# mpkuse/solve_keyframe_pose_graph

Measured on AMD Instinct MI355X. Metric: LM iters/sec + final chi2 vs Ceres, 100k-pose/300k-edge SE(3) graph, higher is better.
Workload: dtype f64

## Files before the change

solve_keyframe_pose_graph_amd/csrc/pgo_internal.hpp:

```cpp
#pragma once
#include <hip/hip_runtime.h>
#include <stdint.h>

#include "pgo_device_math.hpp"

#define PGO_HIPCHK(err, expr)                                                                      \
    do {                                                                                           \
        hipError_t e__ = (expr);                                                                   \
        if (e__ != hipSuccess) {                                                                   \
            (err) = std::string(#expr) + ": " + hipGetErrorString(e__);                            \
            return e__ == hipErrorOutOfMemory ? PGO_ERR_OUT_OF_MEMORY : PGO_ERR_HIP;               \
        }                                                                                          \
    } while (0)

namespace pgo {

constexpr int TILE = 64;
constexpr int REL_DOUBLES = 78;
constexpr int SW_DOUBLES = 86;
constexpr int K1_WAVES = 4;
constexpr int WIN_MAX = 72;
constexpr int WIN_STRIDE = 80;
constexpr int MAX_PARTIALS = 1024;
constexpr int CG_MAX_GRID = 1024;
// ... 70 lines not shown
    double* cen;
    double* d;
    double* Ac;
    double* rc;
    double* yc;
    const int64_t* blk_ptr;
    const int32_t* blk_ab;
    const int64_t* contrib;
    const int32_t* agg_free;
    float* Acf;
};

constexpr int MG_MAX_LEVELS = 12;
constexpr int MG_TILE_ROWS = 32;
struct MgLevelDev {
    int32_t n, n_next, tiles, n_ps;
    int64_t nnzb;
    const int64_t* rowptr; const int32_t* col; double* val;
    const int64_t* g_ptr; const int64_t* g_ent;
    double* Dinv;
    double* pos; double* d;
    const int32_t* parent; const int32_t* agg_ptr; const int4* tile_info; const int2* tile_rows;
    double* r; double* x; double* xt; double* xf;
    float* valf;
    int32_t smoothed, n_w;
    int32_t seg_shift, pad3_;
    const int32_t* ps_rowptr; const int32_t* ps_col; const int32_t* w_rowptr; const int32_t* w_col; const int64_t* psT_ptr; const int64_t* psT_ent;
    double* ps_val; double* w_val;
    double* t; double* u; double* y; const double* zero;
    double* dlump;
    const int32_t* row_of; const int32_t* tr_of;
    const int32_t* ps_row; const int32_t* w_row;
    float* rt_valf; float* r_valf;
    const int2* rt_rows; const int2* rT_rows; const int32_t* rT_col; const int32_t* rT_of_w; const int32_t* ps_of_w;
    int32_t rT_tiles, rT_seg_shift;
    int32_t tile0, tiles_own, rT_row0, rT_row1;
    int32_t su_row0, su_row1, su_ps0, su_ps1, su_w0, su_w1, n_su_prod, pad4_;
    int64_t su_blk0, su_blk1;
    const int32_t* su_prod;
};
struct MgDev {
    int32_t n_levels;
    int32_t n1;
    const int32_t* agg0;
    const int32_t* mem0_ptr; const int32_t* mem0;
    double* d0;
    const int4* blk_tab;
    const double* inv_cnt;
    int32_t a0, a1;
    const int32_t* g0_slots; int32_t n_g0, pad_;
};
constexpr int MG_BLOCK0 = 64;

struct CgDev {
    double* val; float* Lf; double* Dtot; double* b;
    double* x; double* r; double* r2; double* z; double* p; double* p2; double* q;
    double* part_pq;
    double* part_rz;
    int32_t extra_rz;
    int32_t pad_;
    double* scal;
    int32_t* flags;
};

void launch_k1(const GraphDev& G, const double* pose8, const double* sw, bool want_jacobian, double* partials , int* n_partials, hipStream_t st);
void launch_prior(const GraphDev& G, const double* pose8, bool want_jacobian, double* partial_cost , hipStream_t st);
void launch_k2(const GraphDev& G, const LinDev& L, bool want_offdiag, hipStream_t st, const MfDev* F = nullptr );
void launch_scale_init(const GraphDev& G, const LinDev& L, const ScaleDev& Sc, int jacobi_scaling, hipStream_t st);
// ... 93 lines not shown
```

solve_keyframe_pose_graph_amd/csrc/pgo_mg_host.hpp:

```cpp
#pragma once
#include <algorithm>
#include <cmath>
#include <cstdint>
#include <numeric>
#include <utility>
#include <cstdlib>
#include <cstring>
#include <thread>
#include <atomic>
#include <new>
#include <vector>
#include <chrono>
#include <cstdio>
#define PGO_MG_T0() auto t_mg_ = std::chrono::steady_clock::now()
#define PGO_MG_T(what) do { if (pgo_mg::timing()) { auto n_ = std::chrono::steady_clock::now(); std::fprintf(stderr, "[pgo] hierarchy (host): %-28s %7.2f ms\n", what, std::chrono::duration<double, std::milli>(n_ - t_mg_).count()); t_mg_ = n_; } } while (0)

namespace pgo_mg { inline bool& timing() { static thread_local bool on = false; return on; } }

namespace pgo_mg {

struct HostLevel {
    int32_t n = 0;
    std::vector<int64_t> rowptr;
    std::vector<int32_t> col;
    std::vector<int64_t> g_ptr;
    std::vector<int64_t> g_ent;
    std::vector<int32_t> parent;
    std::vector<int32_t> agg_ptr;
    std::vector<int32_t> tile_agg0;
    int seg = 1;
    bool smoothed = false;
    std::vector<int32_t> ps_rowptr, ps_col;
    std::vector<int32_t> w_rowptr, w_col;
    std::vector<int64_t> psT_ptr, psT_ent;
    std::vector<int32_t> ps_of_w;
    std::vector<int32_t> rT_rowptr, rT_col;
    std::vector<int32_t> rT_of_w;
    int rT_seg = 1;
    std::vector<int32_t> own_ptr;
    std::vector<int32_t> tile_ptr;
    bool distributed = false;
};

struct Hierarchy {
    std::vector<HostLevel> L;
    bool fine_smoothed = false;
    HostLevel F;
    std::vector<int32_t> agg0;
    std::vector<int32_t> mem0_ptr, mem0;
    int world = 1;
};

struct Owners {
    const std::vector<uint64_t>* touch_mask = nullptr;
    const std::vector<int32_t>* owner = nullptr;
    int world = 1;
    int32_t dist_min_rows = 8192;
};

struct WEdge { int32_t u, v; double w; };

template <class Fn>
inline void parallel_ranges(int32_t n, int parts, Fn fn) {
    if (parts < 1) parts = 1;
    if (parts == 1 || n < 2048) { fn(0, 0, n); return; }
    std::atomic<bool> helper_failed{false};
    struct Joiner { std::vector<std::thread> th; ~Joiner() { for (std::thread& t : th) if (t.joinable()) t.join(); } } j;
    const int32_t step = (n + parts - 1) / parts;
    for (int k = 0; k + 1 < parts; ++k) {
        const int32_t lo = std::min<int64_t>((int64_t)k * step, n), hi = std::min<int64_t>((int64_t)(k + 1) * step, n);
        bool started = false;
// ... 121 lines not shown
    const std::vector<int32_t>* sc1; const std::vector<int32_t>* sc2;
};

struct BuildCache {
    bool valid = false;
    std::vector<int32_t> agg0_prov; int32_t n1 = 0;
    HostLevel L1prov;
    std::vector<WEdge> rel1;
    std::vector<int32_t> sw_u, sw_v;
    std::vector<int64_t> sw_ptr; std::vector<int32_t> sw_edge;
    std::vector<int32_t> own1_prov;
};

inline void permute_level1(const HostLevel& P, int32_t n, const std::vector<int32_t>& newid, HostLevel& out) {
    std::vector<int32_t> old_of((size_t)n);
    for (int32_t i = 0; i < n; ++i) old_of[newid[i]] = i;
    out.rowptr.assign((size_t)n + 1, 0); out.col.resize(P.col.size()); out.g_ptr.assign(P.col.size() + 1, 0); out.g_ent.resize(P.g_ent.size());
    int64_t kb = 0, ge = 0;
    std::vector<std::pair<int32_t, int64_t>> row;
    for (int32_t r = 0; r < n; ++r) {
        const int32_t o = old_of[r];
        row.clear();
        for (int64_t k = P.rowptr[o]; k < P.rowptr[(size_t)o + 1]; ++k) { const int32_t c = newid[P.col[k]]; row.push_back({c == r ? -1 : c, k}); }
        std::sort(row.begin(), row.end());
        for (const auto& ck : row) {
            out.col[(size_t)kb] = ck.first < 0 ? r : ck.first;
            out.g_ptr[(size_t)kb] = ge;
            for (int64_t g = P.g_ptr[ck.second]; g < P.g_ptr[(size_t)ck.second + 1]; ++g) out.g_ent[(size_t)ge++] = P.g_ent[g];
            ++kb;
        }
        out.rowptr[(size_t)r + 1] = kb;
    }
    out.g_ptr[(size_t)kb] = ge;
}

inline void smoothed_structure(HostLevel& A, HostLevel& B, const std::vector<uint8_t>* ps_keep = nullptr) {
    A.smoothed = true;
    const int32_t n = A.n, nb = B.n;
    const int nth = host_threads();
    auto rows_in_parallel = [&](int32_t rows, std::vector<int32_t>& rowptr_out, std::vector<int32_t>& col_out, auto row_fn ) {
        std::vector<std::vector<int32_t>> part_cols((size_t)nth), part_len((size_t)nth);
        parallel_ranges(rows, nth, [&](int part, int32_t lo, int32_t hi) {
            std::vector<int32_t> tmp, stamp((size_t)nb, -1);
            std::vector<int32_t>& pc = part_cols[(size_t)part]; std::vector<int32_t>& pl = part_len[(size_t)part];
            pl.reserve((size_t)(hi - lo));
            for (int32_t i = lo; i < hi; ++i) { tmp.clear(); row_fn(i, tmp, stamp); pc.insert(pc.end(), tmp.begin(), tmp.end()); pl.push_back((int32_t)tmp.size()); }
        });
        rowptr_out.assign((size_t)rows + 1, 0); col_out.clear();
        int32_t r = 0;
        for (int k = 0; k < nth; ++k) {
            for (int32_t len : part_len[(size_t)k]) { rowptr_out[(size_t)r + 1] = rowptr_out[r] + len; ++r; }
            col_out.insert(col_out.end(), part_cols[(size_t)k].begin(), part_cols[(size_t)k].end());
        }
    };
    rows_in_parallel(n, A.ps_rowptr, A.ps_col, [&](int32_t i, std::vector<int32_t>& tmp, std::vector<int32_t>&) {
        if (A.parent[i] < 0) return;
        for (int64_t k = A.rowptr[i]; k < A.rowptr[(size_t)i + 1]; ++k) { if (ps_keep && !(*ps_keep)[(size_t)k]) continue; const int32_t a = A.parent[A.col[k]]; if (a >= 0) tmp.push_back(a); }
        std::sort(tmp.begin(), tmp.end()); tmp.erase(std::unique(tmp.begin(), tmp.end()), tmp.end());
    });
    rows_in_parallel(n, A.w_rowptr, A.w_col, [&](int32_t i, std::vector<int32_t>& tmp, std::vector<int32_t>& stamp) {
        if (A.parent[i] < 0) return;
        for (int64_t k = A.rowptr[i]; k < A.rowptr[(size_t)i + 1]; ++k) {
            const int32_t j = A.col[k];
            for (int32_t sl = A.ps_rowptr[j]; sl < A.ps_rowptr[(size_t)j + 1]; ++sl) { const int32_t c = A.ps_col[sl]; if (stamp[c] != i) { stamp[c] = i; tmp.push_back(c); } }
        }
        std::sort(tmp.begin(), tmp.end());
// ... 1 lines not shown
    A.psT_ptr.assign((size_t)nb + 1, 0);
    for (int32_t c : A.ps_col) A.psT_ptr[(size_t)c + 1]++;
    for (int32_t a = 0; a < nb; ++a) A.psT_ptr[(size_t)a + 1] += A.psT_ptr[a];
    A.psT_ent.resize(A.ps_col.size());
    { std::vector<int64_t> fill(A.psT_ptr.begin(), A.psT_ptr.end() - 1);
      for (int32_t i = 0; i < n; ++i) for (int32_t sl = A.ps_rowptr[i]; sl < A.ps_rowptr[(size_t)i + 1]; ++sl) A.psT_ent[(size_t)fill[A.ps_col[sl]]++] = ((int64_t)i << 32) | (int64_t)sl; }
    {
        std::vector<int32_t> brow, bcol;
        rows_in_parallel(nb, brow, bcol, [&](int32_t a, std::vector<int32_t>& tmp, std::vector<int32_t>& stamp) {
            std::vector<int32_t> un;
            for (int64_t e = A.psT_ptr[a]; e < A.psT_ptr[(size_t)a + 1]; ++e) {
                const int32_t i = (int32_t)(A.psT_ent[e] >> 32);
                for (int32_t sl = A.w_rowptr[i]; sl < A.w_rowptr[(size_t)i + 1]; ++sl) { const int32_t c = A.w_col[sl]; if (stamp[c] != a) { stamp[c] = a; un.push_back(c); } }
            }
            std::sort(un.begin(), un.end());
            tmp.push_back(a);
            for (int32_t c : un) if (c != a) tmp.push_back(c);
        });
        B.rowptr.assign(brow.begin(), brow.end()); B.col.swap(bcol);
    }
    B.g_ptr.assign(B.col.size() + 1, 0); B.g_ent.clear();
    A.ps_of_w.assign(A.w_col.size(), -1);
    for (int32_t i = 0; i < n; ++i) {
        int32_t ps = A.ps_rowptr[i]; const int32_t pe = A.ps_rowptr[(size_t)i + 1];
        for (int32_t k = A.w_rowptr[i]; k < A.w_rowptr[(size_t)i + 1] && ps < pe; ++k) if (A.w_col[k] == A.ps_col[ps]) A.ps_of_w[(size_t)k] = ps++;
    }
    A.rT_rowptr.assign((size_t)nb + 1, 0);
    for (int32_t c : A.w_col) A.rT_rowptr[(size_t)c + 1]++;
    for (int32_t a = 0; a < nb; ++a) A.rT_rowptr[(size_t)a + 1] += A.rT_rowptr[a];
    A.rT_col.resize(A.w_col.size()); A.rT_of_w.resize(A.w_col.size());
    { std::vector<int32_t> fill(A.rT_rowptr.begin(), A.rT_rowptr.end() - 1);
      for (int32_t i = 0; i < n; ++i) for (int32_t k = A.w_rowptr[i]; k < A.w_rowptr[(size_t)i + 1]; ++k) { const int32_t sl = fill[A.w_col[k]]++; A.rT_col[(size_t)sl] = i; A.rT_of_w[(size_t)k] = sl; } }
    {
        const double mean_row = (double)A.w_col.size() / (double)std::max(1, nb);
        static const double rt_blocks_per_group = []() {
            const char* m = std::getenv("PGO_ENABLE_DEBUG_HOOKS"); const char* e = std::getenv("PGO_DEBUG_RT_SEG_BLOCKS");
            const double v = (m && m[0] == '1' && m[1] == 0 && e) ? std::atof(e) : 0.0; return v >= 1.0 && v <= 64.0 ? v : 5.0; }();
        A.rT_seg = 1;
        while (A.rT_seg < 8 && mean_row > rt_blocks_per_group * A.rT_seg) A.rT_seg *= 2;
    }
}

inline bool build_hierarchy(int64_t N, const std::vector<uint8_t>& node_free, const std::vector<int32_t>& rc1, const std::vector<int32_t>& rc2, const double* rel_w, int rel_w_stride,
                            const std::vector<int32_t>& sc1, const std::vector<int32_t>& sc2, const double* sw_weight ,
                            int passes0, int passes, int dense_max, int tile_rows, int max_levels, Hierarchy& H, bool level0_follows_switchable = true, int level0_block = 0,
                            const LocalContrib* local = nullptr, int smoothed_levels = 0 ,
                            double loop_discount = 0.0 ,
                            BuildCache* cache = nullptr ,
                            const std::vector<int64_t>* fine_rowptr = nullptr, const std::vector<int32_t>* fine_col = nullptr ,
                            const Owners* owners = nullptr ,
                            const std::vector<uint8_t>* fine_keep = nullptr ) {
    H = Hierarchy{};
    const bool owned = owners && owners->touch_mask && owners->owner && owners->world > 1;
    const int world = owned ? owners->world : 1;
    H.world = world;
    auto kf_owner = [&](int64_t g) { return (*owners->owner)[(size_t)g]; };
    PGO_MG_T0();
    const int64_t Er = (int64_t)rc1.size(), Es = (int64_t)sc1.size();
    BuildCache own_cache;
    BuildCache& Cc = (cache && !level0_follows_switchable) ? *cache : own_cache;
    auto collapse = [](const std::vector<WEdge>& in, const std::vector<int32_t>& par) {
        std::vector<WEdge> out;
        out.reserve(in.size());
        for (const WEdge& e : in) { const int32_t u = par[e.u], v = par[e.v]; if (u >= 0 && v >= 0 && u != v) out.push_back({u, v, e.w}); }
        return out;
    };
    if (!Cc.valid) {
        std::vector<WEdge> rel_edges;
        rel_edges.reserve((size_t)Er);
        for (int64_t e = 0; e < Er; ++e) if (node_free[rc1[e]] && node_free[rc2[e]]) {
            const double w = rel_w[(size_t)rel_w_stride * e];
            if (owned && kf_owner(rc1[e]) != kf_owner(rc2[e])) continue;
            if (w * w > 1e-8) rel_edges.push_back({rc1[e], rc2[e], w * w});
// ... 204 lines not shown
    H.mem0.resize((size_t)H.mem0_ptr[n1]);
    { std::vector<int32_t> fill(H.mem0_ptr.begin(), H.mem0_ptr.end() - 1);
      for (int64_t i = 0; i < N; ++i) if (H.agg0[i] >= 0) H.mem0[(size_t)fill[H.agg0[i]]++] = (int32_t)i; }
    PGO_MG_T("numbering + member lists");
    permute_level1(Cc.L1prov, n1, newid_above, H.L[0]);
    PGO_MG_T("permute level 1");
    if (fine_rowptr && fine_col && !local) {
        H.fine_smoothed = true;
        H.F = HostLevel{};
        H.F.n = (int32_t)N; H.F.rowptr = *fine_rowptr; H.F.col = *fine_col; H.F.parent = H.agg0;
        HostLevel B1; B1.n = n1;
        smoothed_structure(H.F, B1, fine_keep);
        H.L[0].rowptr.swap(B1.rowptr); H.L[0].col.swap(B1.col); H.L[0].g_ptr.swap(B1.g_ptr); H.L[0].g_ent.clear();
        PGO_MG_T("fine-level smoothed structure");
    }
    for (size_t l = 0; l + 1 < H.L.size(); ++l) {
        HostLevel& A = H.L[l];
        HostLevel& B = H.L[l + 1];
        if ((int)l < smoothed_levels) { smoothed_structure(A, B); continue; }
        std::vector<std::pair<int64_t, int64_t>> trip;
        trip.reserve(A.col.size());
        for (int32_t r = 0; r < A.n; ++r)
            for (int64_t k = A.rowptr[r]; k < A.rowptr[(size_t)r + 1]; ++k)
                trip.push_back({(int64_t)A.parent[r] * B.n + A.parent[A.col[k]], ((int64_t)r << 32) | k});
        build_blocks(B.n, trip, B);
    }
    PGO_MG_T("upper-level structures");
    for (size_t l = 0; l + 1 < H.L.size(); ++l) {
        HostLevel& Lv = H.L[l];
        const double mean_row = (double)Lv.col.size() / (double)std::max(1, Lv.n);
        int max_agg = 1;
        const int32_t n_next = H.L[l + 1].n;
        for (int32_t a = 0; a < n_next; ++a) max_agg = std::max(max_agg, Lv.agg_ptr[(size_t)a + 1] - Lv.agg_ptr[a]);
        Lv.seg = 1;
        static const double blocks_per_group = []() {
            const char* m = std::getenv("PGO_ENABLE_DEBUG_HOOKS"); const char* e = std::getenv("PGO_DEBUG_SEG_BLOCKS");
            const double v = (m && m[0] == '1' && m[1] == 0 && e) ? std::atof(e) : 0.0; return v >= 1.0 && v <= 64.0 ? v : 5.0; }();
        while (Lv.seg < 8 && mean_row > blocks_per_group * Lv.seg) Lv.seg *= 2;
        while (Lv.seg > 1 && tile_rows / Lv.seg < max_agg) Lv.seg /= 2;
        const int cap = tile_rows / Lv.seg;
        Lv.tile_agg0.clear();
        Lv.tile_agg0.push_back(0);
        int rows = 0;
        const std::vector<int32_t>& up_own = H.L[l + 1].own_ptr;
        int r_cur = 0;
        for (int32_t a = 0; a < n_next; ++a) {
            const int sz = Lv.agg_ptr[(size_t)a + 1] - Lv.agg_ptr[a];
            bool owner_change = false;
            if (owned) while (r_cur + 1 < world && a >= up_own[(size_t)r_cur + 1]) { ++r_cur; owner_change = true; }
            if (rows > 0 && (rows + sz > cap || owner_change)) { Lv.tile_agg0.push_back(a); rows = 0; }
            rows += sz;
        }
        Lv.tile_agg0.push_back(n_next);
        if (owned) {
            const int32_t nt = (int32_t)Lv.tile_agg0.size() - 1;
            Lv.tile_ptr.assign((size_t)world + 1, nt);
            Lv.tile_ptr[0] = 0;
            int32_t t = 0;
            for (int r = 0; r < world; ++r) {
                while (t < nt && Lv.tile_agg0[(size_t)t] < up_own[(size_t)r]) ++t;
                Lv.tile_ptr[(size_t)r] = t;
            }
            Lv.tile_ptr[(size_t)world] = nt;
            for (int r = 0; r < world; ++r) for (int32_t tt = Lv.tile_ptr[(size_t)r]; tt < Lv.tile_ptr[(size_t)r + 1]; ++tt)
                if (Lv.tile_agg0[(size_t)tt] < up_own[(size_t)r] || Lv.tile_agg0[(size_t)tt + 1] > up_own[(size_t)r + 1]) return false;
        }
    }
    return true;
}

struct ExchangePlan {
// ... 214 lines not shown
```

solve_keyframe_pose_graph_amd/csrc/pgo_mg_kernels.hpp:

```cpp

__device__ __forceinline__ int bsr_idx(int row, int col) { return (row >> 1) * 12 + col * 2 + (row & 1); }

__device__ __forceinline__ void mg_row_accumulate(int64_t b, int64_t e, const int32_t* __restrict__ col, const double* __restrict__ val,
                                                  const double* __restrict__ x, int c, double* acc) {
    int64_t k = b;
    for (; k + 4 <= e; k += 4) spmv_chunk<4, false>(col + k, val + (size_t)k * 36, c, x, nullptr, 0.0, acc);
    if (k + 2 <= e) { spmv_chunk<2, false>(col + k, val + (size_t)k * 36, c, x, nullptr, 0.0, acc); k += 2; }
    if (k < e) spmv_chunk<1, false>(col + k, val + (size_t)k * 36, c, x, nullptr, 0.0, acc);
}

template <int U>
__device__ __forceinline__ void mg_chunk_f32(const int32_t* __restrict__ colp, const float* __restrict__ valp, int c, const double* __restrict__ x, double* acc) {
    int32_t col[U];
    float2 v[U][3];
    double xx[U];
#pragma unroll
    for (int u = 0; u < U; ++u) col[u] = colp[u];
#pragma unroll
    for (int u = 0; u < U; ++u) {
        const float2* vp = reinterpret_cast<const float2*>(valp + (size_t)u * 36) + c;
        v[u][0] = vp[0]; v[u][1] = vp[6]; v[u][2] = vp[12];
    }
#pragma unroll
    for (int u = 0; u < U; ++u) xx[u] = x[(size_t)col[u] * 6 + c];
// ... 842 lines not shown
        double x = 0.0;
#pragma unroll
        for (int j = 0; j < 6; ++j) x += Dk[j] * ra[j];
        x_next[(size_t)a * 6 + c] = x;
    }
    MG_TL(6);
}
__global__ __launch_bounds__(384) void mg_dense_solve_kernel(CoarseDev K, MgLevelDev Below, int has_below, double scale, const int32_t* __restrict__ stop) {
    __shared__ double ys[6];
    const int stopped = stop ? *stop : 0;
    const int a = blockIdx.x;
    const int q = threadIdx.x >> 6, lane = threadIdx.x & 63;
    const double2* __restrict__ x = reinterpret_cast<const double2*>(K.rc);
    const float4* __restrict__ Ar = reinterpret_cast<const float4*>(K.Acf + (size_t)(a * 6 + q) * K.nc);
    const int n4 = K.nc >> 2;
    double s = 0.0;
    if (lane < n4) { const float4 u = Ar[lane]; const double2 v = x[2 * lane], w = x[2 * lane + 1]; s = (double)u.x * v.x + (double)u.y * v.y + (double)u.z * w.x + (double)u.w * w.y; }
    if (stopped) return;
#pragma unroll 4
    for (int j = lane + 64; j < n4; j += 64) { const float4 u = Ar[j]; const double2 v = x[2 * j], w = x[2 * j + 1]; s += (double)u.x * v.x + (double)u.y * v.y + (double)u.z * w.x + (double)u.w * w.y; }
    s = wave_sum(s);
    if (lane == 0) { ys[q] = s; K.yc[a * 6 + q] = s; }
    if (!has_below) return;
    __syncthreads();
    double y[6];
#pragma unroll
    for (int k = 0; k < 6; ++k) y[k] = ys[k];
    const int c0 = Below.agg_ptr[a], c1 = Below.agg_ptr[a + 1];
    for (int idx = threadIdx.x; idx < (c1 - c0) * 6; idx += 384) {
        const int i = c0 + idx / 6, k = idx % 6;
        Below.xt[(size_t)i * 6 + k] = Below.x[(size_t)i * 6 + k] + scale * mg_prolong_comp(y, Below.d + (size_t)i * 3, k);
    }
}
template <bool FINE>
__global__ __launch_bounds__(CG_BLOCK) void mg_up_kernel(MgLevelDev A, MgLevelDev Below, int has_below, double scale, const int32_t* __restrict__ stop,
                                                          MgDev M, const double* __restrict__ rfine, double* __restrict__ zfine, double* __restrict__ part_extra,
                                                          const double* __restrict__ xnext = nullptr) {
    __shared__ double xch[CG_BLOCK * 7];
    __shared__ double tb[CG_BLOCK];
    __shared__ double xb[CG_BLOCK];
    const int stopped = stop ? *stop : 0;
    const int q6 = threadIdx.x / 6, c = threadIdx.x % 6;
    const int li = q6 & ((MG_TILE_ROWS >> A.seg_shift) - 1), sg = q6 >> (5 - A.seg_shift);
    double acc2 = 0.0;
    for (int tile = A.tile0 + (int)blockIdx.x; tile < A.tile0 + A.tiles_own; tile += gridDim.x) {
    const int4 ti = A.tile_info[tile];
    const bool expl = xnext != nullptr;
    const int2 rb = expl ? A.rt_rows[tile * MG_TILE_ROWS + li] : A.tile_rows[tile * MG_TILE_ROWS + li];
    if (stopped) return;
    const int i0 = ti.z, i1 = ti.w;
    const int row = i0 + li;
    const bool rowlive = row < i1;
    const bool live = rowlive && sg == 0;
    double rv = 0.0, xv = 0.0;
    double Dk[6] = {0.0, 0.0, 0.0, 0.0, 0.0, 0.0};
    int c0 = 0, c1 = 0;
    if (live) {
        rv = A.r[(size_t)row * 6 + c]; xv = expl ? A.y[(size_t)row * 6 + c] : A.xt[(size_t)row * 6 + c];
        if (!expl) {
            const double2* Dp = reinterpret_cast<const double2*>(A.Dinv + (size_t)row * 36 + c * 6);
            const double2 u0 = Dp[0], u1 = Dp[1], u2 = Dp[2];
            Dk[0] = u0.x; Dk[1] = u0.y; Dk[2] = u1.x; Dk[3] = u1.y; Dk[4] = u2.x; Dk[5] = u2.y;
        }
    }
    if (has_below) { c0 = Below.agg_ptr[i0]; c1 = Below.agg_ptr[i1]; }
    const int idx0 = threadIdx.x;
    int ch = 0, chk = 0, chp = 0; double chx = 0.0, chd[3] = {0.0, 0.0, 0.0};
    const bool first = has_below && idx0 < (c1 - c0) * 6;
    if (first) {
        ch = c0 + idx0 / 6; chk = idx0 % 6;
        chp = Below.parent[ch]; chx = Below.x[(size_t)ch * 6 + chk];
        chd[0] = Below.d[(size_t)ch * 3]; chd[1] = Below.d[(size_t)ch * 3 + 1]; chd[2] = Below.d[(size_t)ch * 3 + 2];
    }
    constexpr int FT = FINE ? (MG_TILE_ROWS * 8 * 3 + CG_BLOCK - 1) / CG_BLOCK : 1;
    int fn[FT], fa[FT]; double fd[FT][3]; double2 fz[FT];
    int fcnt = 0;
    if (FINE) {
        const int e0 = M.mem0_ptr[i0];
        fcnt = (M.mem0_ptr[i1] - e0) * 3;
#pragma unroll
        for (int tt = 0; tt < FT; ++tt) {
            const int idx = threadIdx.x + tt * CG_BLOCK;
            fn[tt] = -1;
            if (idx < fcnt) {
                const int n = M.mem0[e0 + idx / 3], j = idx % 3;
                fn[tt] = n * 3 + j; fa[tt] = M.agg0[n] - i0;
                fd[tt][0] = M.d0[(size_t)n * 3]; fd[tt][1] = M.d0[(size_t)n * 3 + 1]; fd[tt][2] = M.d0[(size_t)n * 3 + 2];
                fz[tt] = reinterpret_cast<const double2*>(zfine)[(size_t)n * 3 + j];
            }
        }
    }
    double acc[6] = {0.0, 0.0, 0.0, 0.0, 0.0, 0.0};
    if (expl) { if (rowlive) { int kb, ke; mg_split_row(rb, sg, A.seg_shift, kb, ke); mg_row_accumulate_f32(kb, ke, A.w_col, A.rt_valf, xnext, c, acc); } }
    else MG_ROW_PRODUCT(tile, A.xt);
    double* mine = xch + (size_t)threadIdx.x * 7;
#pragma unroll
    for (int q = 0; q < 6; ++q) mine[q] = acc[q];
    __syncthreads();
    if (expl) {
        if (live) {
            const double x = xv + scale * mg_gather_row(xch, li, c, A.seg_shift);
            A.xf[(size_t)row * 6 + c] = x;
            xb[threadIdx.x] = x;
        }
    } else {
        if (live) tb[threadIdx.x] = rv - mg_gather_row(xch, li, c, A.seg_shift);
        __syncthreads();
        if (live) {
            const double* ta = tb + (threadIdx.x - c);
            double x = xv;
#pragma unroll
            for (int j = 0; j < 6; ++j) x += Dk[j] * ta[j];
            A.xf[(size_t)row * 6 + c] = x;
            xb[threadIdx.x] = x;
        }
    }
    if (FINE) {
        __syncthreads();
        if (live) acc2 += scale * rv * xb[threadIdx.x];
#pragma unroll
        for (int tt = 0; tt < FT; ++tt) {
            if (fn[tt] < 0) continue;
            const int j = fn[tt] % 3;
            const double* y = xb + (size_t)fa[tt] * 6;
            const double b0 = scale * mg_prolong_comp(y, fd[tt], 2 * j), b1 = scale * mg_prolong_comp(y, fd[tt], 2 * j + 1);
            reinterpret_cast<double2*>(zfine)[fn[tt]] = make_double2(fz[tt].x + b0, fz[tt].y + b1);
        }
        __syncthreads();
        continue;
    }
    if (!has_below) return;
    __syncthreads();
    if (first) Below.xt[(size_t)ch * 6 + chk] = chx + scale * mg_prolong_comp(xb + (size_t)(chp - i0) * 6, chd, chk);
    for (int idx = threadIdx.x + CG_BLOCK; idx < (c1 - c0) * 6; idx += CG_BLOCK) {
// ... 208 lines not shown
    else if (g1 == 0) {}
    else if (nl == 1) hipLaunchKernelGGL(mg_restrict0_kernel, dim3(g1), dim3(CG_BLOCK), 0, st, M, r, K.rc, (double*)nullptr, (const double*)nullptr, stop);
    else hipLaunchKernelGGL(mg_restrict0_kernel, dim3(g1), dim3(CG_BLOCK), 0, st, M, r, levels[0].r, levels[0].x, (const double*)levels[0].Dinv, stop);
    for (int l = 1; l < nl; ++l) {
        MgLevelDev A = levels[l - 1];
        xchg(0, l);
        if (hook_failed) return;
        if (A.smoothed && A.rt_valf) {
            const unsigned g = (unsigned)(A.tiles_own + A.rT_tiles);
            if (g == 0) continue;
            if (l + 1 == nl) hipLaunchKernelGGL(mg_sdown_kernel, dim3(g), dim3(CG_BLOCK), 0, st, A, K.rc, (double*)nullptr, (const double*)nullptr, stop);
            else hipLaunchKernelGGL(mg_sdown_kernel, dim3(g), dim3(CG_BLOCK), 0, st, A, levels[l].r, levels[l].x, (const double*)levels[l].Dinv, stop);
            continue;
        }
        if (A.tiles_own == 0) continue;
        if (A.smoothed) {
            hipLaunchKernelGGL(mg_smooth_step_kernel, dim3((unsigned)A.tiles_own), dim3(CG_BLOCK), 0, st, A, (const double*)A.r, (const double*)A.x, A.t, (const double*)nullptr, (const double*)nullptr, A.u, prolong_scale, stop);
            A.r = A.t; A.x = A.u;
        }
        if (l + 1 == nl) hipLaunchKernelGGL(mg_down_kernel, dim3((unsigned)A.tiles_own), dim3(CG_BLOCK), 0, st, A, K.rc, (double*)nullptr, (const double*)nullptr, stop);
        else hipLaunchKernelGGL(mg_down_kernel, dim3((unsigned)A.tiles_own), dim3(CG_BLOCK), 0, st, A, levels[l].r, levels[l].x, (const double*)levels[l].Dinv, stop);
    }
    auto below_of = [&](int idx) { MgLevelDev B = levels[idx]; if (B.smoothed) B.x = const_cast<double*>(B.zero); return B; };
    auto expl_at = [&](int idx) { return idx >= 0 && levels[idx].smoothed && levels[idx].rt_valf != nullptr; };
    xchg(0, nl);
    if (hook_failed) return;
    hipLaunchKernelGGL(mg_dense_solve_kernel, dim3((unsigned)K.n_agg), dim3(384), 0, st, K, nl >= 2 ? below_of(nl - 2) : levels[0], nl >= 2 && !expl_at(nl - 2) ? 1 : 0, scale, stop);
    const bool fused = C.extra_rz > 0;
    const unsigned g0 = (unsigned)cg_grid(G);
    for (int l = nl - 1; l >= 1; --l) {
        MgLevelDev A = levels[l - 1];
        xchg(1, l);
        if (hook_failed) return;
        if (A.tiles_own == 0) continue;
        if (expl_at(l - 1)) {
            const double* xn = l + 1 == nl ? (const double*)K.yc : (const double*)levels[l].xf;
            if (l == 1 && fused) hipLaunchKernelGGL(mg_up_kernel<true>, dim3((unsigned)(A.tiles_own < MAX_PARTIALS ? A.tiles_own : MAX_PARTIALS)), dim3(CG_BLOCK), 0, st, A, A, 0, scale, stop, M, r, z, part_rz + g0, xn);
            else hipLaunchKernelGGL(mg_up_kernel<false>, dim3((unsigned)A.tiles_own), dim3(CG_BLOCK), 0, st, A, l >= 2 ? below_of(l - 2) : levels[0], l >= 2 && !expl_at(l - 2) ? 1 : 0, scale, stop, M, r, z, part_rz, xn);
            continue;
        }
        if (A.smoothed) {
            hipLaunchKernelGGL(mg_smooth_step_kernel, dim3((unsigned)A.tiles_own), dim3(CG_BLOCK), 0, st, A, (const double*)nullptr, (const double*)A.xt, (double*)nullptr, (const double*)A.x, (const double*)A.xt, A.y, prolong_scale, stop);
            A.xt = A.y;
        }
        if (l == 1 && fused) hipLaunchKernelGGL(mg_up_kernel<true>, dim3((unsigned)(A.tiles_own < MAX_PARTIALS ? A.tiles_own : MAX_PARTIALS)), dim3(CG_BLOCK), 0, st, A, A, 0, scale, stop, M, r, z, part_rz + g0, (const double*)nullptr);
        else hipLaunchKernelGGL(mg_up_kernel<false>, dim3((unsigned)A.tiles_own), dim3(CG_BLOCK), 0, st, A, l >= 2 ? below_of(l - 2) : levels[0], l >= 2 && !expl_at(l - 2) ? 1 : 0, scale, stop, M, r, z, part_rz, (const double*)nullptr);
    }
    xchg(2, 1);
    if (hook_failed) return;
    if (fine) hipLaunchKernelGGL(mg_prolong0s_kernel, dim3(g0), dim3(CG_BLOCK), 0, st, G, *fine, (const double*)(nl == 1 ? K.yc : levels[0].xf), r, z, part_rz, scale, stop);
    else if (!fused) hipLaunchKernelGGL(mg_prolong0_kernel, dim3(g0), dim3(CG_BLOCK), 0, st, G, M, (const double*)(nl == 1 ? K.yc : levels[0].xf), r, z, part_rz, scale, stop);
}
```

solve_keyframe_pose_graph_amd/csrc/pgo_multigrid.hip:

```cpp
#include <algorithm>
#include <atomic>
#include <cmath>
#include <cstdio>
#include <cstring>
#include <memory>
#include <thread>
#include <vector>

#include "pgo_handle.hpp"

namespace pgo {

struct MgPrepared {
    bool ok = false;
    pgo_mg::Hierarchy H;
    std::vector<double> inv_cnt;
    std::vector<int32_t> pi32; std::vector<int64_t> pi64; size_t nf64 = 0;
    enum Pool { I32, I64, F64 };
    struct Reloc { void* field; Pool pool; size_t off; };
    std::vector<Reloc> reloc;
    MgDev M{}; MgLevelDev levels[MG_MAX_LEVELS]{};
    bool fine = false; MgLevelDev fineF{}, fineT{};
    std::vector<pgo_mg::ExchangePlan> plans; std::vector<LevelPlanDev> lvl_plan;
    pgo_mg::SetupPlans setup; std::vector<SetupPlanDev> su_plan;
// ... 112 lines not shown
                    started = true;
                } catch (...) {}
            }
            pgo_mg::build_level_plans(H, OW, p->rank(), Q.plans);
            if (started) { worker.join(); if (worker_failed.load()) throw std::bad_alloc(); }
            else if (want_setup) pgo_mg::build_setup_plans(H, p->rank(), p->world(), grc1, grc2, rel_off, gsc1, gsc2, sw_off, Q.setup);
        }
        if (ok) {
            const int32_t n1g = (int32_t)H.mem0_ptr.size() - 1;
            inv_cnt.resize((size_t)n1g);
            for (int32_t a = 0; a < n1g; ++a) inv_cnt[a] = 1.0 / (double)std::max(1, H.mem0_ptr[a + 1] - H.mem0_ptr[a]);
            agg0_l.resize((size_t)N); mem0_ptr_l.assign((size_t)n1g + 1, 0);
            for (int64_t l = 0; l < N; ++l) { agg0_l[l] = p->h_node_free[l] ? H.agg0[p->l2g[l]] : -1; if (agg0_l[l] >= 0) mem0_ptr_l[(size_t)agg0_l[l] + 1]++; }
            for (int32_t a = 0; a < n1g; ++a) mem0_ptr_l[(size_t)a + 1] += mem0_ptr_l[a];
            mem0_l.resize((size_t)mem0_ptr_l[n1g]);
            std::vector<int32_t> fillm(mem0_ptr_l.begin(), mem0_ptr_l.end() - 1);
            for (int64_t l = 0; l < N; ++l) if (agg0_l[l] >= 0) mem0_l[(size_t)fillm[agg0_l[l]]++] = (int32_t)l;
        }
    }
    Q.ok = ok;
    if (!ok) return PGO_OK;
    const std::vector<int32_t>& A0 = p->local_ids ? agg0_l : H.agg0;
    const std::vector<int32_t>& M0P = p->local_ids ? mem0_ptr_l : H.mem0_ptr;
    const std::vector<int32_t>& M0 = p->local_ids ? mem0_l : H.mem0;
    const int nl = (int)H.L.size();
    const bool dist = H.world > 1;
    const int rank = p->rank();
    const bool expl = p->opt.mg_explicit_transfer != 0 || p->local_ids;
    std::vector<int32_t>& pi32 = Q.pi32; std::vector<int64_t>& pi64 = Q.pi64;
    {
        size_t n32 = A0.size() + M0P.size() + M0.size() + (size_t)((N + MG_BLOCK0 - 1) / MG_BLOCK0) * MG_BLOCK0 * 4 + 64, n64 = 0;
        for (const pgo_mg::HostLevel& A : H.L) {
            const size_t tiles = A.tile_agg0.empty() ? 0 : A.tile_agg0.size() - 1;
            n32 += 3 * A.col.size() + A.parent.size() + A.agg_ptr.size() + tiles * (4 + 2 * (size_t)MG_TILE_ROWS) + A.ps_rowptr.size() + 2 * A.ps_col.size() + A.w_rowptr.size() + 5 * A.w_col.size() + (A.smoothed ? tiles * 2 * (size_t)MG_TILE_ROWS + ((size_t)A.rT_rowptr.size() / 4 + 2) * 2 * (size_t)MG_TILE_ROWS : 0) + 16;
            n64 += A.rowptr.size() + A.g_ptr.size() + A.g_ent.size() + A.psT_ptr.size() + A.psT_ent.size();
        }
        if (H.fine_smoothed) {
            const pgo_mg::HostLevel& F = H.F;
            n32 += F.col.size() + F.ps_rowptr.size() + 4 * F.ps_col.size() + F.w_rowptr.size() + 2 * F.w_col.size() + ((size_t)H.L[0].n / 4 + 2) * 2 * (size_t)MG_TILE_ROWS + 16;
            n64 += F.rowptr.size() + F.col.size() + F.psT_ptr.size() + F.psT_ent.size();
        }
        pi32.reserve(n32); pi64.reserve(n64);
    }
    auto rel = [&](void* field, MgPrepared::Pool pool, size_t off) { if (field) Q.reloc.push_back({field, pool, off}); };
    auto put32 = [&](const std::vector<int32_t>& v, void* field) { const size_t o = pi32.size(); pi32.insert(pi32.end(), v.begin(), v.end()); rel(field, MgPrepared::I32, o); return o; };
    auto put64 = [&](const std::vector<int64_t>& v, void* field) { rel(field, MgPrepared::I64, pi64.size()); pi64.insert(pi64.end(), v.begin(), v.end()); };
    auto take = [&](size_t cnt, void* field) { const size_t o = Q.nf64; Q.nf64 += (cnt + 1) & ~(size_t)1; rel(field, MgPrepared::F64, o); return o; };
    auto align32 = [&](size_t k) { while (pi32.size() % k) pi32.push_back(0); };
    MgDev& M = Q.M;
    M.n_levels = nl; M.n1 = H.L[0].n;
    M.a0 = dist ? H.L[0].own_ptr[(size_t)rank] : 0; M.a1 = dist ? H.L[0].own_ptr[(size_t)rank + 1] : H.L[0].n;
    const size_t o_agg0 = put32(A0, &M.agg0); put32(M0P, &M.mem0_ptr); put32(M0, &M.mem0);
    bool have_tab = !p->local_ids && !H.fine_smoothed;
    if (have_tab) {
        const int64_t runs = (N + MG_BLOCK0 - 1) / MG_BLOCK0;
        std::vector<int32_t> tab((size_t)runs * MG_BLOCK0 * 4);
        for (size_t k = 0; k < tab.size(); k += 4) { tab[k] = -1; tab[k + 1] = -1; tab[k + 2] = -1; tab[k + 3] = 0; }
        std::vector<int> fill((size_t)runs, 0);
        const int32_t n1h = (int32_t)H.mem0_ptr.size() - 1;
        for (int32_t a = 0; a < n1h && have_tab; ++a) {
            const int32_t m0 = H.mem0_ptr[a], m1 = H.mem0_ptr[a + 1];
            if (m1 <= m0) continue;
            const int64_t run = H.mem0[m0] / MG_BLOCK0;
            if (m1 - m0 > 8 || fill[run] >= MG_BLOCK0) { have_tab = false; break; }
            uint32_t w[2] = {0xffffffffu, 0xffffffffu};
            for (int32_t m = m0; m < m1; ++m) {
                if (H.mem0[m] / MG_BLOCK0 != run) { have_tab = false; break; }
// ... 53 lines not shown
                            const int32_t* b = A.col.data() + A.rowptr[j] + 1; const int32_t* e = A.col.data() + A.rowptr[(size_t)j + 1];
                            const int32_t* f = std::lower_bound(b, e, i);
                            if (f != e && *f == i) t = f - A.col.data();
                        }
                        tr_of[(size_t)k] = (int32_t)t;
                    }
            });
            put32(row_of, &D.row_of); put32(tr_of, &D.tr_of);
        }
        {
            std::vector<int32_t> info;
            for (size_t tt = 0; tt + 1 < A.tile_agg0.size(); ++tt) { const int32_t a0 = A.tile_agg0[tt], a1 = A.tile_agg0[tt + 1]; info.insert(info.end(), {a0, a1, A.agg_ptr[a0], A.agg_ptr[a1]}); }
            align32(4);
            put32(info, &D.tile_info);
            std::vector<int32_t> rows;
            for (size_t tt = 0; tt + 1 < A.tile_agg0.size(); ++tt) {
                const int32_t i0 = A.agg_ptr[A.tile_agg0[tt]], i1 = A.agg_ptr[A.tile_agg0[tt + 1]];
                for (int li = 0; li < MG_TILE_ROWS; ++li) { const int32_t r = i0 + li; rows.push_back(r < i1 ? (int32_t)A.rowptr[r] : 0); rows.push_back(r < i1 ? (int32_t)A.rowptr[r + 1] : 0); }
            }
            put32(rows, &D.tile_rows);
        }
        put64(A.rowptr, &D.rowptr); put64(A.g_ptr, &D.g_ptr); put64(A.g_ent, &D.g_ent);
        take(A.col.size() * 36, &D.val); take((size_t)A.n * 36, &D.Dinv); take((size_t)A.n * 3, &D.pos); take((size_t)A.n * 3, &D.d);
        take((size_t)A.n * 6, &D.r); take((size_t)A.n * 6, &D.x); take((size_t)A.n * 6, &D.xt); take((size_t)A.n * 6, &D.xf);
        take((A.col.size() * 36 + 1) / 2, &D.valf);
        if (A.smoothed) {
            put32(A.ps_rowptr, &D.ps_rowptr); put32(A.ps_col, &D.ps_col); put32(A.w_rowptr, &D.w_rowptr); put32(A.w_col, &D.w_col);
            put64(A.psT_ptr, &D.psT_ptr); put64(A.psT_ent, &D.psT_ent);
            put32(row_index(A.ps_rowptr), &D.ps_row); put32(row_index(A.w_rowptr), &D.w_row);
            take(A.ps_col.size() * 36, &D.ps_val); take(A.w_col.size() * 36, &D.w_val);
            take((size_t)A.n * 6, &D.t); take((size_t)A.n * 6, &D.u); take((size_t)A.n * 6, &D.y); take((size_t)A.n * 6, &D.zero);
            {
                put32(A.rT_col, expl ? &D.rT_col : nullptr); put32(A.rT_of_w, expl ? &D.rT_of_w : nullptr); put32(A.ps_of_w, expl ? &D.ps_of_w : nullptr);
                std::vector<int32_t> rows;
                for (size_t tt = 0; tt + 1 < A.tile_agg0.size(); ++tt) {
                    const int32_t i0 = A.agg_ptr[A.tile_agg0[tt]], i1 = A.agg_ptr[A.tile_agg0[tt + 1]];
                    for (int li = 0; li < MG_TILE_ROWS; ++li) { const int32_t r = i0 + li; rows.push_back(r < i1 ? A.w_rowptr[r] : 0); rows.push_back(r < i1 ? A.w_rowptr[(size_t)r + 1] : 0); }
                }
                align32(2);
                put32(rows, expl ? &D.rt_rows : nullptr);
                const int seg_shift = A.rT_seg >= 8 ? 3 : A.rT_seg >= 4 ? 2 : A.rT_seg >= 2 ? 1 : 0;
                const int rpt = MG_TILE_ROWS >> seg_shift;
                const int32_t nb0 = D.rT_row0, nb = D.rT_row1;
                const int rT_tiles = (nb - nb0 + rpt - 1) / rpt;
                if (expl) { D.rT_tiles = rT_tiles; D.rT_seg_shift = seg_shift; }
                rows.clear();
                for (int tt = 0; tt < rT_tiles; ++tt)
                    for (int li = 0; li < MG_TILE_ROWS; ++li) { const int32_t r = nb0 + tt * rpt + li; const bool in = li < rpt && r < nb; rows.push_back(in ? A.rT_rowptr[r] : 0); rows.push_back(in ? A.rT_rowptr[(size_t)r + 1] : 0); }
                put32(rows, expl ? &D.rT_rows : nullptr);
                take((A.w_col.size() * 36 + 1) / 2, expl ? &D.rt_valf : nullptr); take((A.w_col.size() * 36 + 1) / 2, expl ? &D.r_valf : nullptr);
            }
        }
    }
    Q.lvl_plan.assign(Q.plans.size(), LevelPlanDev{});
    for (size_t l = 0; l < Q.plans.size(); ++l) { put32(Q.plans[l].send_idx, &Q.lvl_plan[l].send_idx); put32(Q.plans[l].recv_idx, &Q.lvl_plan[l].recv_idx); }
    if (Q.setup.first_whole > 0) {
        const pgo_mg::HostLevel& L1 = H.L[0];
        std::vector<int32_t> g0_slots;
        for (size_t k = 0; k + 1 < L1.g_ptr.size(); ++k) if (L1.g_ptr[k + 1] > L1.g_ptr[k]) g0_slots.push_back((int32_t)k);
        put32(g0_slots, &M.g0_slots); M.n_g0 = (int32_t)g0_slots.size();
        const pgo_mg::HostLevel& W = H.L[(size_t)Q.setup.first_whole];
        Q.fw_row0 = W.own_ptr[(size_t)rank]; Q.fw_row1 = W.own_ptr[(size_t)rank + 1];
        Q.fw_blk0 = W.rowptr[(size_t)Q.fw_row0]; Q.fw_blk1 = W.rowptr[(size_t)Q.fw_row1];
    }
    Q.su_plan.assign(Q.setup.val.size(), SetupPlanDev{});
    for (size_t l = 0; l < Q.setup.val.size(); ++l) {
        SetupPlanDev& so = Q.su_plan[l];
        const pgo_mg::BlockPlan& B = Q.setup.val[l];
        put32(B.x.send_idx, &so.val_send); put32(B.dst, &so.val_dst); put32(B.sum_ptr, &so.val_sum_ptr); put32(B.sum_src, &so.val_sum_src);
        if (l < Q.setup.ps.size()) {
            put32(Q.setup.ps[l].send_idx, &so.ps_send); put32(Q.setup.ps[l].recv_idx, &so.ps_recv); put32(Q.setup.rv[l].send_idx, &so.rv_send); put32(Q.setup.rv[l].recv_idx, &so.rv_recv);
            const bool smoothed = H.L[l].smoothed;
            put32(Q.setup.prod[l], smoothed ? &Q.levels[l].su_prod : nullptr);
// ... 354 lines not shown

int build_mg(pgo_problem* p) {
    MgState& m = p->mg;
    m.active = false;
    if (!m.built) return PGO_OK;
    int rc;
    if ((rc = mg_fresh_install(p)) != PGO_OK) return rc;
    if (!m.built) return PGO_OK;
    const double t_build0 = now_s();
    if ((rc = p->local_ids ? maybe_regroup(p) : regroup_install(p)) != PGO_OK) return rc;
    if (!m.built) return PGO_OK;
    if (p->opt.verbosity > 1) std::fprintf(stderr, "[pgo] multigrid: build_mg past the regroup at %.2f ms\n", (now_s() - t_build0) * 1e3);
    if (m.geometry_epoch != p->lin_epoch) {
        if (p->local_ids) {
            launch_mg_geometry0_sum(p->G, m.M, m.levels, p->d_pose[p->cur].p, p->st);
            if ((rc = allreduce(p, m.levels[0].pos, (size_t)m.M.n1 * 3, 0)) != PGO_OK) return rc;
            launch_mg_geometry_finish(p->G, m.M, m.levels, p->d_pose[p->cur].p, p->st);
        } else launch_mg_geometry(p->G, m.M, m.levels, p->d_pose[p->cur].p, p->st);
        m.geometry_epoch = p->lin_epoch;
    }
    int32_t* fail = p->d_cinfo.p;
    HIPCHK(p, hipMemsetAsync(fail, 0, sizeof(int32_t), p->st));
    bool hoff_valid = !p->built_mf;
    if (p->built_mf && p->d_Hoff.cap >= (size_t)(p->G.rel.Epad + p->G.sw.Epad) * 36) {
        if (p->hoff_epoch != p->lin_epoch) { p->L.Hoff = p->d_Hoff.p; launch_k2_offdiag(p->G, p->L, p->st); p->hoff_epoch = p->lin_epoch; }
        hoff_valid = true;
    }
    if ((rc = mg_operators(p, fail, hoff_valid, false, t_build0)) != PGO_OK) return rc;
    if (debug_break_coarse()) launch_coarse_negate(p->K, p->st);
    int32_t h = 1;
    HIPCHK(p, hipMemcpyAsync(&h, fail, sizeof(h), hipMemcpyDeviceToHost, p->st));
    HIPCHK(p, hipStreamSynchronize(p->st));
    m.active = h == 0;
    const int t1 = m.levels[0].tiles;
    p->C.extra_rz = (m.active && !p->local_ids && !m.fine && m.M.n_levels >= 2 && (t1 <= MAX_PARTIALS || t1 >= 2 * MAX_PARTIALS)) ? std::min<int>(t1, MAX_PARTIALS) : 0;
    if (p->opt.verbosity > 0 && h != 0) std::fprintf(stderr, "[pgo] multigrid: a coarse block is not positive definite at radius %.1e -> off for this iteration\n", p->radius);
    if (p->opt.verbosity > 1) std::fprintf(stderr, "[pgo] multigrid: operators of LM iteration %d built in %.2f ms\n", p->iteration, (now_s() - t_build0) * 1e3);
    return PGO_OK;
}

}
```

Measured before the change: 112.4.

## Give explicit-R prolongation its own row tiling with lane-group splitting

The prolongation (up) kernel for explicitly smoothed levels now uses its own tile layout over owned rows instead of the aggregate-based tiles. Each row's nonzeros are pre-split into lane groups chosen from the mean row length, so several thread groups share one long row. The goal is better load balance and occupancy in the f32 row-product of the up sweep. In exchange it adds host-side tile tables, more template instantiations for the fused fine path, and changes to the tile counts that feed the partial-reduction sizing.

Measured after the change: 114.1 (median of 6 runs). Within noise of the previous version (+1.5%).

```diff
diff --git a/solve_keyframe_pose_graph_amd/csrc/pgo_internal.hpp b/solve_keyframe_pose_graph_amd/csrc/pgo_internal.hpp
--- a/solve_keyframe_pose_graph_amd/csrc/pgo_internal.hpp
+++ b/solve_keyframe_pose_graph_amd/csrc/pgo_internal.hpp
@@ -126,8 +126,9 @@
     const int32_t* row_of; const int32_t* tr_of;
     const int32_t* ps_row; const int32_t* w_row;
     float* rt_valf; float* r_valf;
-    const int2* rt_rows; const int2* rT_rows; const int32_t* rT_col; const int32_t* rT_of_w; const int32_t* ps_of_w;
+    const int2* rt_up_rows; const int2* rT_rows; const int32_t* rT_col; const int32_t* rT_of_w; const int32_t* ps_of_w;
     int32_t rT_tiles, rT_seg_shift;
+    int32_t rt_up_tiles, rt_up_seg_shift, rt_up_row0, rt_up_row1;
     int32_t tile0, tiles_own, rT_row0, rT_row1;
     int32_t su_row0, su_row1, su_ps0, su_ps1, su_w0, su_w1, n_su_prod, pad4_;
     int64_t su_blk0, su_blk1;
diff --git a/solve_keyframe_pose_graph_amd/csrc/pgo_mg_host.hpp b/solve_keyframe_pose_graph_amd/csrc/pgo_mg_host.hpp
--- a/solve_keyframe_pose_graph_amd/csrc/pgo_mg_host.hpp
+++ b/solve_keyframe_pose_graph_amd/csrc/pgo_mg_host.hpp
@@ -37,6 +37,7 @@
     std::vector<int32_t> rT_rowptr, rT_col;
     std::vector<int32_t> rT_of_w;
     int rT_seg = 1;
+    int rt_up_seg = 1;
     std::vector<int32_t> own_ptr;
     std::vector<int32_t> tile_ptr;
     bool distributed = false;
@@ -224,6 +225,17 @@
         out.rowptr[(size_t)r + 1] = kb;
     }
     out.g_ptr[(size_t)kb] = ge;
+}
+
+inline int lane_groups(double mean_row, double blocks_per_group) {
+    int g = 1;
+    while (g < 8 && mean_row > blocks_per_group * g) g *= 2;
+    return g;
+}
+inline double debug_blocks_per_group(const char* name, double dflt = 5.0) {
+    const char* m = std::getenv("PGO_ENABLE_DEBUG_HOOKS"); const char* e = std::getenv(name);
+    const double v = (m && m[0] == '1' && m[1] == 0 && e) ? std::atof(e) : 0.0;
+    return v >= 1.0 && v <= 64.0 ? v : dflt;
 }
 
 inline void smoothed_structure(HostLevel& A, HostLevel& B, const std::vector<uint8_t>* ps_keep = nullptr) {
@@ -291,13 +303,27 @@
     { std::vector<int32_t> fill(A.rT_rowptr.begin(), A.rT_rowptr.end() - 1);
       for (int32_t i = 0; i < n; ++i) for (int32_t k = A.w_rowptr[i]; k < A.w_rowptr[(size_t)i + 1]; ++k) { const int32_t sl = fill[A.w_col[k]]++; A.rT_col[(size_t)sl] = i; A.rT_of_w[(size_t)k] = sl; } }
     {
-        const double mean_row = (double)A.w_col.size() / (double)std::max(1, nb);
-        static const double rt_blocks_per_group = []() {
-            const char* m = std::getenv("PGO_ENABLE_DEBUG_HOOKS"); const char* e = std::getenv("PGO_DEBUG_RT_SEG_BLOCKS");
-            const double v = (m && m[0] == '1' && m[1] == 0 && e) ? std::atof(e) : 0.0; return v >= 1.0 && v <= 64.0 ? v : 5.0; }();
-        A.rT_seg = 1;
-        while (A.rT_seg < 8 && mean_row > rt_blocks_per_group * A.rT_seg) A.rT_seg *= 2;
-    }
+        static const double rt_blocks_per_group = debug_blocks_per_group("PGO_DEBUG_RT_SEG_BLOCKS"), up_blocks_per_group = debug_blocks_per_group("PGO_DEBUG_RT_UP_SEG_BLOCKS", 6.0);
+        A.rT_seg = lane_groups((double)A.w_col.size() / (double)std::max(1, nb), rt_blocks_per_group);
+        A.rt_up_seg = lane_groups((double)A.w_col.size() / (double)std::max(1, n), up_blocks_per_group);
+    }
+}
+
+template <class Ptr>
+inline std::vector<int32_t> group_tiles(const Ptr* rowptr, int32_t row0, int32_t row1, int tile_rows, int groups) {
+    const int rpt = tile_rows / groups;
+    const int32_t tiles = row1 > row0 ? (row1 - row0 + rpt - 1) / rpt : 0;
+    std::vector<int32_t> slots((size_t)tiles * tile_rows * 2, 0);
+    for (int32_t t = 0; t < tiles; ++t)
+        for (int li = 0; li < rpt && row0 + t * rpt + li < row1; ++li) {
+            const int32_t r = row0 + t * rpt + li;
+            const int32_t b = (int32_t)rowptr[r], e = (int32_t)rowptr[(size_t)r + 1], part = (e - b + groups - 1) / groups;
+            for (int g = 0; g < groups; ++g) {
+                int32_t* s = &slots[((size_t)t * tile_rows + (size_t)g * rpt + li) * 2];
+                s[0] = std::min(b + g * part, e); s[1] = std::min(b + (g + 1) * part, e);
+            }
+        }
+    return slots;
 }
 
 inline bool build_hierarchy(int64_t N, const std::vector<uint8_t>& node_free, const std::vector<int32_t>& rc1, const std::vector<int32_t>& rc2, const double* rel_w, int rel_w_stride,
@@ -568,11 +594,8 @@
         int max_agg = 1;
         const int32_t n_next = H.L[l + 1].n;
         for (int32_t a = 0; a < n_next; ++a) max_agg = std::max(max_agg, Lv.agg_ptr[(size_t)a + 1] - Lv.agg_ptr[a]);
-        Lv.seg = 1;
-        static const double blocks_per_group = []() {
-            const char* m = std::getenv("PGO_ENABLE_DEBUG_HOOKS"); const char* e = std::getenv("PGO_DEBUG_SEG_BLOCKS");
-            const double v = (m && m[0] == '1' && m[1] == 0 && e) ? std::atof(e) : 0.0; return v >= 1.0 && v <= 64.0 ? v : 5.0; }();
-        while (Lv.seg < 8 && mean_row > blocks_per_group * Lv.seg) Lv.seg *= 2;
+        static const double blocks_per_group = debug_blocks_per_group("PGO_DEBUG_SEG_BLOCKS");
+        Lv.seg = lane_groups(mean_row, blocks_per_group);
         while (Lv.seg > 1 && tile_rows / Lv.seg < max_agg) Lv.seg /= 2;
         const int cap = tile_rows / Lv.seg;
         Lv.tile_agg0.clear();
diff --git a/solve_keyframe_pose_graph_amd/csrc/pgo_mg_kernels.hpp b/solve_keyframe_pose_graph_amd/csrc/pgo_mg_kernels.hpp
--- a/solve_keyframe_pose_graph_amd/csrc/pgo_mg_kernels.hpp
+++ b/solve_keyframe_pose_graph_amd/csrc/pgo_mg_kernels.hpp
@@ -898,7 +898,7 @@
         Below.xt[(size_t)i * 6 + k] = Below.x[(size_t)i * 6 + k] + scale * mg_prolong_comp(y, Below.d + (size_t)i * 3, k);
     }
 }
-template <bool FINE>
+template <bool FINE, int FT = 1>
 __global__ __launch_bounds__(CG_BLOCK) void mg_up_kernel(MgLevelDev A, MgLevelDev Below, int has_below, double scale, const int32_t* __restrict__ stop,
                                                           MgDev M, const double* __restrict__ rfine, double* __restrict__ zfine, double* __restrict__ part_extra,
                                                           const double* __restrict__ xnext = nullptr) {
@@ -906,15 +906,19 @@
     __shared__ double tb[CG_BLOCK];
     __shared__ double xb[CG_BLOCK];
     const int stopped = stop ? *stop : 0;
+    const bool expl = xnext != nullptr;
+    const int ss = expl ? A.rt_up_seg_shift : A.seg_shift, rpt = MG_TILE_ROWS >> ss;
     const int q6 = threadIdx.x / 6, c = threadIdx.x % 6;
-    const int li = q6 & ((MG_TILE_ROWS >> A.seg_shift) - 1), sg = q6 >> (5 - A.seg_shift);
+    const int li = q6 & (rpt - 1), sg = q6 >> (5 - ss);
     double acc2 = 0.0;
-    for (int tile = A.tile0 + (int)blockIdx.x; tile < A.tile0 + A.tiles_own; tile += gridDim.x) {
-    const int4 ti = A.tile_info[tile];
-    const bool expl = xnext != nullptr;
-    const int2 rb = expl ? A.rt_rows[tile * MG_TILE_ROWS + li] : A.tile_rows[tile * MG_TILE_ROWS + li];
+    const int ntiles = expl ? A.rt_up_tiles : A.tiles_own;
+    for (int t = (int)blockIdx.x; t < ntiles; t += gridDim.x) {
+    const int tile = A.tile0 + t;
+    int i0, i1;
+    int2 rb;
+    if (expl) { i0 = A.rt_up_row0 + t * rpt; i1 = min(i0 + rpt, A.rt_up_row1); rb = A.rt_up_rows[t * MG_TILE_ROWS + q6]; }
+    else { const int4 ti = A.tile_info[tile]; i0 = ti.z; i1 = ti.w; rb = A.tile_rows[tile * MG_TILE_ROWS + li]; }
     if (stopped) return;
-    const int i0 = ti.z, i1 = ti.w;
     const int row = i0 + li;
     const bool rowlive = row < i1;
     const bool live = rowlive && sg == 0;
@@ -938,7 +942,6 @@
         chp = Below.parent[ch]; chx = Below.x[(size_t)ch * 6 + chk];
         chd[0] = Below.d[(size_t)ch * 3]; chd[1] = Below.d[(size_t)ch * 3 + 1]; chd[2] = Below.d[(size_t)ch * 3 + 2];
     }
-    constexpr int FT = FINE ? (MG_TILE_ROWS * 8 * 3 + CG_BLOCK - 1) / CG_BLOCK : 1;
     int fn[FT], fa[FT]; double fd[FT][3]; double2 fz[FT];
     int fcnt = 0;
     if (FINE) {
@@ -957,7 +960,7 @@
         }
     }
     double acc[6] = {0.0, 0.0, 0.0, 0.0, 0.0, 0.0};
-    if (expl) { if (rowlive) { int kb, ke; mg_split_row(rb, sg, A.seg_shift, kb, ke); mg_row_accumulate_f32(kb, ke, A.w_col, A.rt_valf, xnext, c, acc); } }
+    if (expl) { if (rowlive) mg_row_accumulate_f32(rb.x, rb.y, A.w_col, A.rt_valf, xnext, c, acc); }
     else MG_ROW_PRODUCT(tile, A.xt);
     double* mine = xch + (size_t)threadIdx.x * 7;
 #pragma unroll
@@ -965,7 +968,7 @@
     __syncthreads();
     if (expl) {
         if (live) {
-            const double x = xv + scale * mg_gather_row(xch, li, c, A.seg_shift);
+            const double x = xv + scale * mg_gather_row(xch, li, c, ss);
             A.xf[(size_t)row * 6 + c] = x;
             xb[threadIdx.x] = x;
         }
@@ -1240,18 +1243,25 @@
         MgLevelDev A = levels[l - 1];
         xchg(1, l);
         if (hook_failed) return;
+        if (expl_at(l - 1)) {
+            if (A.rt_up_tiles == 0) continue;
+            const double* xn = l + 1 == nl ? (const double*)K.yc : (const double*)levels[l].xf;
+            if (l == 1 && fused) {
+                const dim3 grid((unsigned)(A.rt_up_tiles < MAX_PARTIALS ? A.rt_up_tiles : MAX_PARTIALS));
+                const int rows = MG_TILE_ROWS >> A.rt_up_seg_shift;
+                if (rows <= 8) hipLaunchKernelGGL((mg_up_kernel<true, 1>), grid, dim3(CG_BLOCK), 0, st, A, A, 0, scale, stop, M, r, z, part_rz + g0, xn);
+                else if (rows <= 16) hipLaunchKernelGGL((mg_up_kernel<true, 2>), grid, dim3(CG_BLOCK), 0, st, A, A, 0, scale, stop, M, r, z, part_rz + g0, xn);
+                else hipLaunchKernelGGL((mg_up_kernel<true, 4>), grid, dim3(CG_BLOCK), 0, st, A, A, 0, scale, stop, M, r, z, part_rz + g0, xn);
+            }
+            else hipLaunchKernelGGL(mg_up_kernel<false>, dim3((unsigned)A.rt_up_tiles), dim3(CG_BLOCK), 0, st, A, l >= 2 ? below_of(l - 2) : levels[0], l >= 2 && !expl_at(l - 2) ? 1 : 0, scale, stop, M, r, z, part_rz, xn);
+            continue;
+        }
         if (A.tiles_own == 0) continue;
-        if (expl_at(l - 1)) {
-            const double* xn = l + 1 == nl ? (const double*)K.yc : (const double*)levels[l].xf;
-            if (l == 1 && fused) hipLaunchKernelGGL(mg_up_kernel<true>, dim3((unsigned)(A.tiles_own < MAX_PARTIALS ? A.tiles_own : MAX_PARTIALS)), dim3(CG_BLOCK), 0, st, A, A, 0, scale, stop, M, r, z, part_rz + g0, xn);
-            else hipLaunchKernelGGL(mg_up_kernel<false>, dim3((unsigned)A.tiles_own), dim3(CG_BLOCK), 0, st, A, l >= 2 ? below_of(l - 2) : levels[0], l >= 2 && !expl_at(l - 2) ? 1 : 0, scale, stop, M, r, z, part_rz, xn);
-            continue;
-        }
         if (A.smoothed) {
             hipLaunchKernelGGL(mg_smooth_step_kernel, dim3((unsigned)A.tiles_own), dim3(CG_BLOCK), 0, st, A, (const double*)nullptr, (const double*)A.xt, (double*)nullptr, (const double*)A.x, (const double*)A.xt, A.y, prolong_scale, stop);
             A.xt = A.y;
         }
-        if (l == 1 && fused) hipLaunchKernelGGL(mg_up_kernel<true>, dim3((unsigned)(A.tiles_own < MAX_PARTIALS ? A.tiles_own : MAX_PARTIALS)), dim3(CG_BLOCK), 0, st, A, A, 0, scale, stop, M, r, z, part_rz + g0, (const double*)nullptr);
+        if (l == 1 && fused) hipLaunchKernelGGL((mg_up_kernel<true, 4>), dim3((unsigned)(A.tiles_own < MAX_PARTIALS ? A.tiles_own : MAX_PARTIALS)), dim3(CG_BLOCK), 0, st, A, A, 0, scale, stop, M, r, z, part_rz + g0, (const double*)nullptr);
         else hipLaunchKernelGGL(mg_up_kernel<false>, dim3((unsigned)A.tiles_own), dim3(CG_BLOCK), 0, st, A, l >= 2 ? below_of(l - 2) : levels[0], l >= 2 && !expl_at(l - 2) ? 1 : 0, scale, stop, M, r, z, part_rz, (const double*)nullptr);
     }
     xchg(2, 1);
diff --git a/solve_keyframe_pose_graph_amd/csrc/pgo_multigrid.hip b/solve_keyframe_pose_graph_amd/csrc/pgo_multigrid.hip
--- a/solve_keyframe_pose_graph_amd/csrc/pgo_multigrid.hip
+++ b/solve_keyframe_pose_graph_amd/csrc/pgo_multigrid.hip
@@ -168,7 +168,7 @@
         size_t n32 = A0.size() + M0P.size() + M0.size() + (size_t)((N + MG_BLOCK0 - 1) / MG_BLOCK0) * MG_BLOCK0 * 4 + 64, n64 = 0;
         for (const pgo_mg::HostLevel& A : H.L) {
             const size_t tiles = A.tile_agg0.empty() ? 0 : A.tile_agg0.size() - 1;
-            n32 += 3 * A.col.size() + A.parent.size() + A.agg_ptr.size() + tiles * (4 + 2 * (size_t)MG_TILE_ROWS) + A.ps_rowptr.size() + 2 * A.ps_col.size() + A.w_rowptr.size() + 5 * A.w_col.size() + (A.smoothed ? tiles * 2 * (size_t)MG_TILE_ROWS + ((size_t)A.rT_rowptr.size() / 4 + 2) * 2 * (size_t)MG_TILE_ROWS : 0) + 16;
+            n32 += 3 * A.col.size() + A.parent.size() + A.agg_ptr.size() + tiles * (4 + 2 * (size_t)MG_TILE_ROWS) + A.ps_rowptr.size() + 2 * A.ps_col.size() + A.w_rowptr.size() + 5 * A.w_col.size() + (A.smoothed ? ((size_t)A.n / 4 + 2) * 2 * (size_t)MG_TILE_ROWS + ((size_t)A.rT_rowptr.size() / 4 + 2) * 2 * (size_t)MG_TILE_ROWS : 0) + 16;
             n64 += A.rowptr.size() + A.g_ptr.size() + A.g_ent.size() + A.psT_ptr.size() + A.psT_ent.size();
         }
         if (H.fine_smoothed) {
@@ -288,13 +288,12 @@
             take((size_t)A.n * 6, &D.t); take((size_t)A.n * 6, &D.u); take((size_t)A.n * 6, &D.y); take((size_t)A.n * 6, &D.zero);
             {
                 put32(A.rT_col, expl ? &D.rT_col : nullptr); put32(A.rT_of_w, expl ? &D.rT_of_w : nullptr); put32(A.ps_of_w, expl ? &D.ps_of_w : nullptr);
-                std::vector<int32_t> rows;
-                for (size_t tt = 0; tt + 1 < A.tile_agg0.size(); ++tt) {
-                    const int32_t i0 = A.agg_ptr[A.tile_agg0[tt]], i1 = A.agg_ptr[A.tile_agg0[tt + 1]];
-                    for (int li = 0; li < MG_TILE_ROWS; ++li) { const int32_t r = i0 + li; rows.push_back(r < i1 ? A.w_rowptr[r] : 0); rows.push_back(r < i1 ? A.w_rowptr[(size_t)r + 1] : 0); }
-                }
+                const int up_shift = A.rt_up_seg >= 8 ? 3 : A.rt_up_seg >= 4 ? 2 : A.rt_up_seg >= 2 ? 1 : 0;
+                const int32_t u0 = A.agg_ptr[A.tile_agg0[(size_t)D.tile0]], u1 = A.agg_ptr[A.tile_agg0[(size_t)(D.tile0 + D.tiles_own)]];
+                std::vector<int32_t> rows = pgo_mg::group_tiles(A.w_rowptr.data(), u0, u1, MG_TILE_ROWS, 1 << up_shift);
+                if (expl) { D.rt_up_tiles = (int32_t)(rows.size() / (2 * MG_TILE_ROWS)); D.rt_up_seg_shift = up_shift; D.rt_up_row0 = u0; D.rt_up_row1 = u1; }
                 align32(2);
-                put32(rows, expl ? &D.rt_rows : nullptr);
+                put32(rows, expl ? &D.rt_up_rows : nullptr);
                 const int seg_shift = A.rT_seg >= 8 ? 3 : A.rT_seg >= 4 ? 2 : A.rT_seg >= 2 ? 1 : 0;
                 const int rpt = MG_TILE_ROWS >> seg_shift;
                 const int32_t nb0 = D.rT_row0, nb = D.rT_row1;
@@ -715,7 +714,7 @@
     HIPCHK(p, hipMemcpyAsync(&h, fail, sizeof(h), hipMemcpyDeviceToHost, p->st));
     HIPCHK(p, hipStreamSynchronize(p->st));
     m.active = h == 0;
-    const int t1 = m.levels[0].tiles;
+    const int t1 = m.levels[0].rt_valf ? m.levels[0].rt_up_tiles : m.levels[0].tiles;
     p->C.extra_rz = (m.active && !p->local_ids && !m.fine && m.M.n_levels >= 2 && (t1 <= MAX_PARTIALS || t1 >= 2 * MAX_PARTIALS)) ? std::min<int>(t1, MAX_PARTIALS) : 0;
     if (p->opt.verbosity > 0 && h != 0) std::fprintf(stderr, "[pgo] multigrid: a coarse block is not positive definite at radius %.1e -> off for this iteration\n", p->radius);
     if (p->opt.verbosity > 1) std::fprintf(stderr, "[pgo] multigrid: operators of LM iteration %d built in %.2f ms\n", p->iteration, (now_s() - t_build0) * 1e3);
```
